# GRIPS-code/pyLBL

Measured on AMD Instinct MI355X. Metric: line×gridpoint Voigt evals/sec (whole job; per GPU: evals_per_s_per_gpu; spectra/sec: spectra_per_s), higher is better.
Workload: dtype f64; 1 GPU; BASELINE config 'target': 1 level(s) per GPU, H2O+CO2, grid 1-5000 cm-1 at 0.001 cm-1 (5000000 points), cut_off 25, remove_pedestal=False; levels_total=1, atmosphere=surface, output=gas, parallelism=levels sharded

## Files before the change

### pylbl_amd/csrc/accumulate.h

```cpp
#pragma once

#include <hip/hip_runtime.h>

#include "line_prep.h"
#include "voigt_profile.h"

namespace lbl {

struct Tiling
{
    int aligned;
    int per_cell;
    int length;
    int n_tiles;
};

__host__ __device__ inline void tile_bounds(const Tiling & t, int tile, int n_per_v, int n,
                                            long long & i0, long long & i1)
{
    if (t.aligned)
    {
        const int cell = tile/t.per_cell;
        const int sub = tile - cell*t.per_cell;
        i0 = (long long)cell*n_per_v + (long long)sub*t.length;
// ... 13 lines not shown
{
    int lo, a1, c1, c2, a2, hi;
    int f1, f2;
};

__host__ __device__ inline double tile_centre(int v0, double dv, long long i0, long long i1)
{
    const double v_lo = (double)v0 + (double)i0*dv;
    const double v_hi = (double)v0 + (double)i1*dv;
    return 0.5*(v_lo + v_hi);
}

#ifndef LBL_WING_GROUP
#define LBL_WING_GROUP 8
#endif
#ifndef LBL_FAR_TERMS
#define LBL_FAR_TERMS 21
#define LBL_FAR_RATIO 4.
#endif
constexpr int kFarTerms = LBL_FAR_TERMS;
constexpr double kFarRatio = LBL_FAR_RATIO;

struct alignas(16) WorkItem
{
    int tile;
    int part, parts;
    int slot;
};

struct AccumulateArgs
{
    const LineWing * wing;
    const LineCore * core;
    const TileSchedule * schedule;
    const LevelScalars * levels;
    const WorkItem * items;
    const double * far_series;
    const int * wing_bounds;
    int wing_batches;
    double * partial;
    long long partial_slots;
    double * k;
    long long level_stride;
    long long n_lines;
    Tiling tiling;
    int n_tiles;
    int n;
    int v0, n_per_v;
    double dv;
    double v0_real;
    int scale_density;
    int accumulate;
    int inner_everywhere;
#ifdef LBL_ABLATE
    int ablate;
#endif
};

#ifdef LBL_ABLATE
#define LBL_ABLATED(a, bits) (((a).ablate & (bits)) != 0)
#else
#define LBL_ABLATED(a, bits) false
#endif

}

#include "accumulate_lines.h"

namespace lbl {

__device__ __forceinline__ void share_of(int j0, int j1, int part, int parts, float inverse,
                                         int unit_shift, int & begin, int & end)
{
    const int units = (j1 - j0) >> unit_shift;
    const float scale = (float)units;
    const int cut0 = min((int)(scale*((float)part*inverse)), units);
    const int cut1 = min((int)(scale*((float)(part + 1)*inverse)), units);
    begin = j0 + (cut0 << unit_shift);
    end = (part + 1 == parts) ? j1 : j0 + (cut1 << unit_shift);
}

template <int P>
__device__ __forceinline__ void accumulate_tile(const AccumulateArgs & a)
{
    __shared__ double partial[4][P][64];
    const int wave = __builtin_amdgcn_readfirstlane(threadIdx.x >> 6);
    const int lane = threadIdx.x & 63;
    const int level = blockIdx.y;
    const WorkItem item = a.items[blockIdx.x];
    const int tile = item.tile;
    long long first_point, last_point;
    tile_bounds(a.tiling, tile, a.n_per_v, a.n, first_point, last_point);
    const int i0 = (int)first_point, i1 = (int)last_point;
    const TileSchedule sc = a.schedule[(long long)level*a.n_tiles + tile];
    const LineWing * __restrict__ wing = a.wing + (long long)level*a.n_lines;
    const LineCore * __restrict__ core = a.core + (long long)level*a.n_lines;

    double v[P], acc[P];
    double * slab = &partial[wave][0][0];
    __shared__ InnerStage inner_stage[4];
    const double first_index = (double)(i0 + lane);
#pragma unroll
    for (int p = 0; p < P; ++p)
    {
        const double step = (first_index + (double)(p*64))*a.dv;
        v[p] = a.v0_real + step;
        acc[p] = 0.;
    }

    const int piece = item.part*4 + wave, pieces = item.parts*4;
    GeneralList g;
    int fa0, fa1, fb0, fb1, e;
    const bool clipped_in_groups = !a.inner_everywhere && !LBL_ABLATED(a, 64);
    const float inverse = 1.f/(float)pieces;
    share_of(sc.lo, sc.a1, piece, pieces, inverse, clipped_in_groups ? 3 : 0, g.begin[0], e);
    g.count[0] = e - g.begin[0];
    share_of(sc.c1, sc.c2, piece, pieces, inverse, 0, g.begin[1], e);
    g.count[1] = e - g.begin[1];
    share_of(sc.a2, sc.hi, piece, pieces, inverse, clipped_in_groups ? 3 : 0, g.begin[2], e);
    g.count[2] = e - g.begin[2];
    share_of(sc.f1, sc.c1, piece, pieces, inverse, 2, fa0, fa1);
    share_of(sc.c2, sc.f2, piece, pieces, inverse, 2, fb0, fb1);
    g.begin[3] = fa0 + ((fa1 - fa0) & ~3);
    g.count[3] = (fa1 - fa0) & 3;
    g.begin[4] = fb0 + ((fb1 - fb0) & ~3);
    g.count[4] = (fb1 - fb0) & 3;
    if (LBL_ABLATED(a, 4)) { g.count[0] = 0; g.count[2] = 0; }
    if (LBL_ABLATED(a, 8)) { g.count[3] = 0; g.count[4] = 0; }
    if (LBL_ABLATED(a, 16)) { g.count[1] = 0; }
    if (!LBL_ABLATED(a, 2))
    {
        int batches = 1;
        if (P == 4)
        {
            const int * __restrict__ wb = a.wing_bounds + level*kWingBounds;
            const int bound[kWingBounds] = {wb[0], wb[1], wb[2], wb[3]};
            batches = __builtin_amdgcn_readfirstlane(min(wing_batches(bound), a.wing_batches));
        }
        fast_ranges<P>(wing, fa0, fa1, fb0, fb1, batches, v, acc);
    }
    bool slab_in_use = false;
    if (!LBL_ABLATED(a, 1))
    {
        GeneralList walk = g;
        if (clipped_in_groups)
        {
            clipped_ranges<P>(wing, core, g.begin[0], g.count[0], g.begin[2], g.count[2], i0, i1,
                              lane, v, acc);
            walk.count[0] = walk.count[2] = 0;
        }
        general_ranges<P>(wing, core, walk, i0, i1, lane, v, acc);
        if (!LBL_ABLATED(a, 32) && a.levels[level].inner_possible != 0.)
        {
            GeneralList inner = g;
            if (!a.inner_everywhere)
            {
                inner.count[0] = inner.count[2] = inner.count[3] = inner.count[4] = 0;
            }
            slab_in_use = inner_ranges(wing, core, inner, inner_stage[wave], i0, i1, a.v0,
                                       a.n_per_v, a.dv, lane, slab, P);
        }
    }

#pragma unroll
    for (int p = 0; p < P; ++p)
    {
        partial[wave][p][lane] = slab_in_use ? partial[wave][p][lane] + acc[p] : acc[p];
    }
    __syncthreads();

    const bool add_series = a.far_series != nullptr && item.part == 0;
    const double * __restrict__ series = a.far_series +
        ((long long)level*a.n_tiles + tile)*kFarTerms;
    const double u0 = tile_centre(a.v0, a.dv, first_point, last_point);
    auto series_at = [&](double vv) {
        const double u = vv - u0;
        double value = series[kFarTerms - 1];
#pragma unroll
        for (int k = kFarTerms - 2; k >= 0; --k)
        {
            value = __builtin_fma(value, u, series[k]);
        }
        return value;
    };
// ... 110 lines not shown
```

### pylbl_amd/csrc/accumulate_lines.h

```cpp
#pragma once

namespace lbl {

template <int P>
__device__ __forceinline__ void fast_ranges(const LineWing * __restrict__ wing,
                                            int a0, int a1, int b0, int b1, int batches,
                                            const double (&v)[P], double (&acc)[P])
{
    const int qa = (a1 - a0) >> 2;
    const int quads = qa + ((b1 - b0) >> 2);
    int q = 0;
#if LBL_WING_GROUP == 8
    auto eight = [&](int at, WingTerm (&l)[8]) {
        const int ja = at < qa ? a0 + 4*at : b0 + 4*(at - qa);
        const int jb = (at + 1) < qa ? a0 + 4*(at + 1) : b0 + 4*(at + 1 - qa);
#pragma unroll
        for (int i = 0; i < 4; ++i)
        {
            const LineWing wa = wing[ja + i], wb = wing[jb + i];
            l[i] = WingTerm{wa.centre, wa.g2, wa.bl};
            l[4 + i] = WingTerm{wb.centre, wb.g2, wb.bl};
        }
    };
    if (P == 4 && batches > 1)
    {
        const int eights = quads >> 1;
        for (int o = 0; o < eights; )
        {
            const int stop = min(o + batches, eights);
            double num[P], den[P];
            {
                WingTerm l[8];
                eight(2*o, l);
#pragma unroll
                for (int p = 0; p < P; ++p)
                {
                    wing_eight(v[p], l, num[p], den[p]);
                }
            }
// ... 10 lines not shown
                    den[p] = den[p]*t;
                }
            }
#pragma unroll
            for (int p = 0; p < P; ++p)
            {
                acc[p] = __builtin_fma(num[p], rcp_newton(den[p]), acc[p]);
            }
        }
        q = 2*eights;
    }
    for (; q + 2 <= quads; q += 2)
    {
        WingTerm l[8];
        eight(q, l);
#pragma unroll
        for (int p = 0; p < P; ++p)
        {
            acc[p] = lorentz_eight(v[p], l, acc[p]);
        }
    }
#endif
    for (; q < quads; ++q)
    {
        const int j = q < qa ? a0 + 4*q : b0 + 4*(q - qa);
        const LineWing l1 = wing[j], l2 = wing[j + 1], l3 = wing[j + 2], l4 = wing[j + 3];
#pragma unroll
        for (int p = 0; p < P; ++p)
        {
            acc[p] = lorentz_four(v[p], l1.centre, l1.g2, l1.bl, l2.centre, l2.g2, l2.bl,
                                  l3.centre, l3.g2, l3.bl, l4.centre, l4.g2, l4.bl, acc[p]);
        }
    }
}

__device__ __forceinline__ unsigned row_bits(int lo, int hi, int rows)
{
    lo = max(lo, 0);
    hi = min(hi, rows - 1);
    return lo > hi ? 0u : ((2u << hi) - 1u) & ~((1u << lo) - 1u);
}

__device__ __forceinline__ unsigned rows_meeting(int a, int b, int i0, int rows)
{
    return b < a ? 0u : row_bits((a - i0) >> 6, (b - i0) >> 6, rows);
}

__device__ __forceinline__ unsigned rows_inside(int a, int b, int i0, int rows)
{
    return b < a ? 0u : row_bits((a - i0 + 63) >> 6, (b - 63 - i0) >> 6, rows);
}

template <int P>
__device__ __forceinline__ void general_line(const LineWing & l, const LineCore & c,
                                             int i0, int i1, int lane,
                                             const double (&v)[P], double (&acc)[P])
{
    const unsigned in_window = rows_meeting(l.first, l.last, i0, P);
    if (in_window == 0)
    {
        return;
    }
    const unsigned all_region_one = rows_inside(c.mid_first, c.mid_last, i0, P) &
                                    ~rows_meeting(c.hole_first, c.hole_last, i0, P);
    const unsigned near_core = rows_meeting(c.core_first, c.core_last, i0, P);
    const double rsqrpi = 0.56418958354775628695;
    const double yq = c.y*c.y;
    const double a0 = yq + 0.5;
    const double d0 = a0*a0;
    const double d2 = yq + yq - 1.;
    const double r1_scale = c.amp*rsqrpi*c.y;
#pragma unroll
    for (int p = 0; p < P; ++p)
    {
        if (!(in_window & (1u << p)))
        {
            continue;
        }
        const int r0 = i0 + p*64;
        const double d = v[p] - l.centre;
        if (all_region_one & (1u << p))
        {
            const double xi = d*c.repwid;
            const double xq = xi*xi;
            acc[p] += r1_scale*(a0 + xq)*rcp_newton(__builtin_fma(xq, d2 + xq, d0));
            continue;
        }
        const int i = r0 + lane;
        const bool inside = (i >= l.first) && (i <= l.last);
        double value;
        if (!(near_core & (1u << p)))
        {
            value = l.bl*rcp_newton(__builtin_fma(d, d, l.g2));
        }
        else
        {
            const double xi = d*c.repwid;
            const double abx = fabs(xi);
            const double xq = abx*abx;
            const bool far = abx >= c.xlim0;
            const bool mid = !far && abx >= c.xlim1;
            value = 0.;
            if (__any(far))
            {
                const double wing = l.bl*rcp_newton(__builtin_fma(d, d, l.g2));
                value = far ? wing : value;
            }
            if (__any(mid))
            {
                const double w4 = r1_scale*(a0 + xq)*
                                  rcp_newton(__builtin_fma(xq, d2 + xq, d0));
                value = mid ? w4 : value;
            }
        }
        acc[p] += inside ? value : 0.;
    }
}

struct GeneralList
{
    int begin[5];
    int count[5];
};

__device__ __forceinline__ int general_index(const GeneralList & g, int k)
{
    if (k < g.count[0]) return g.begin[0] + k;
    k -= g.count[0];
    if (k < g.count[1]) return g.begin[1] + k;
    k -= g.count[1];
    if (k < g.count[2]) return g.begin[2] + k;
    k -= g.count[2];
    if (k < g.count[3]) return g.begin[3] + k;
    k -= g.count[3];
    return g.begin[4] + k;
}

constexpr int kInnerQueue = 32;
constexpr int kInnerList = 128;

struct InnerStage
{
    int first[kInnerQueue];
    int begin[kInnerQueue], end[kInnerQueue];
    double centre[kInnerQueue], repwid[kInnerQueue], y[kInnerQueue], amp[kInnerQueue];
// ... 135 lines not shown
                    const int rank = __builtin_amdgcn_mbcnt_hi(
                        (unsigned)(mask >> 32), __builtin_amdgcn_mbcnt_lo((unsigned)mask, 0));
                    stage.list[c][count[c] + rank] = record;
                }
                count[c] += __builtin_popcountll(mask);
            }
        }
#pragma unroll
        for (int c = 0; c < kInnerClasses; ++c)
        {
            if (count[c] >= 64 || (drain && count[c] > 0))
            {
                const int now = min(count[c], 64);
                if (c == 0) inner_evaluate<0>(stage, now, i0, v0, dv, lane, slab);
                if (c == 1) inner_evaluate<1>(stage, now, i0, v0, dv, lane, slab);
                if (c == 2) inner_evaluate<2>(stage, now, i0, v0, dv, lane, slab);
                count[c] -= now;
                const unsigned short rest = stage.list[c][64 + lane];
                if (lane < count[c])
                {
                    stage.list[c][lane] = rest;
                }
            }
        }
        if (drain)
        {
            break;
        }
    }
    return true;
}

template <int P>
__device__ __forceinline__ void core_line(const LineWing & l, const LineCore & c, unsigned rows,
                                          const double (&v)[P], double (&acc)[P])
{
    const double rsqrpi = 0.56418958354775628695;
    const double yq = c.y*c.y;
    const double a0 = yq + 0.5;
    const double d0 = a0*a0;
    const double d2 = yq + yq - 1.;
    const double r1_scale = c.amp*rsqrpi*c.y;
    const unsigned special = rows | (rows >> 8);
#pragma unroll
    for (int p = 0; p < P; ++p)
    {
        const double d = v[p] - l.centre;
        if (__builtin_expect(!(special & (1u << p)), 1))
        {
            acc[p] = __builtin_fma(l.bl, rcp_newton(__builtin_fma(d, d, l.g2)), acc[p]);
        }
        else if (rows & (1u << p))
        {
            const double xi = d*c.repwid;
            const double xq = xi*xi;
            acc[p] += r1_scale*(a0 + xq)*rcp_newton(__builtin_fma(xq, d2 + xq, d0));
        }
        else
        {
            const double xi = d*c.repwid;
            const double abx = fabs(xi);
            const double xq = abx*abx;
            const bool far = abx >= c.xlim0;
            const bool mid = !far && abx >= c.xlim1;
            double value = 0.;
            if (__any(far))
            {
                const double wing = l.bl*rcp_newton(__builtin_fma(d, d, l.g2));
                value = far ? wing : value;
            }
            if (__any(mid))
            {
                const double w4 = r1_scale*(a0 + xq)*
                                  rcp_newton(__builtin_fma(xq, d2 + xq, d0));
                value = mid ? w4 : value;
            }
            acc[p] += value;
        }
    }
}

template <int P>
__device__ __forceinline__ void core_lines(const LineWing * __restrict__ wing,
                                           const LineCore * __restrict__ core,
                                           int begin, int count, int i0, int lane,
                                           const double (&v)[P], double (&acc)[P])
{
    for (int base = 0; base < count; base += 64)
    {
        const int n = min(64, count - base);
        const LineCore * __restrict__ mine = core + begin + base + min(lane, n - 1);
        const unsigned all_region_one = rows_inside(mine->mid_first, mine->mid_last, i0, P) &
                                        ~rows_meeting(mine->hole_first, mine->hole_last, i0, P);
        const unsigned near_core = rows_meeting(mine->core_first, mine->core_last, i0, P);
        const unsigned packed = all_region_one | (near_core << 8);
        for (int k = 0; k < n; k += 2)
        {
            const int j = begin + base + k;
            const LineWing la = wing[j], lb = wing[j + 1];
            const LineCore ca = core[j], cb = core[j + 1];
            core_line<P>(la, ca, (unsigned)__builtin_amdgcn_readlane((int)packed, k), v, acc);
            core_line<P>(lb, cb, (unsigned)__builtin_amdgcn_readlane((int)packed, k + 1), v, acc);
        }
    }
}

template <int P>
__device__ __forceinline__ void general_ranges(const LineWing * __restrict__ wing,
                                               const LineCore * __restrict__ core,
                                               const GeneralList & g, int i0, int i1, int lane,
                                               const double (&v)[P], double (&acc)[P])
{
    core_lines<P>(wing, core, g.begin[1], g.count[1] & ~1, i0, lane, v, acc);
    GeneralList rest = g;
    rest.begin[1] = g.begin[1] + (g.count[1] & ~1);
    rest.count[1] = g.count[1] & 1;
    const int total = rest.count[0] + rest.count[1] + rest.count[2] + rest.count[3] + rest.count[4];
    for (int k = 0; k < total; ++k)
    {
        const int j = general_index(rest, k);
        const LineWing l = wing[j];
        const LineCore c = core[j];
        general_line<P>(l, c, i0, i1, lane, v, acc);
    }
}

template <int P>
__device__ __forceinline__ void clipped_ranges(const LineWing * __restrict__ wing,
                                               const LineCore * __restrict__ core,
                                               int begin0, int count0, int begin1, int count1,
                                               int i0, int i1, int lane,
                                               const double (&v)[P], double (&acc)[P])
{
    const int total = count0 + count1;
    int k = 0;
    while (k < total)
    {
        const int j = k < count0 ? begin0 + k : begin1 + (k - count0);
        const bool room = k < count0 ? k + 8 <= count0 : k + 8 <= total;
        if (room)
        {
            const LineWing * __restrict__ mine = wing + j + (lane & 7);
            const int my_first = mine->first, my_last = mine->last;
            WingTerm l[8];
#pragma unroll
            for (int i = 0; i < 8; ++i)
            {
                const LineWing w = wing[j + i];
                l[i] = WingTerm{w.centre, w.g2, w.bl};
            }
            const int first = __builtin_amdgcn_readfirstlane(my_first);
            const int last = __builtin_amdgcn_readfirstlane(my_last);
            if (__ballot(my_first != first || my_last != last) == 0)
            {
#pragma unroll
                for (int p = 0; p < P; ++p)
                {
                    const int r0 = i0 + p*64;
                    if (last < r0 || first > r0 + 63)
                    {
                        continue;
                    }
                    const int i = r0 + lane;
                    const double sum = lorentz_eight(v[p], l, acc[p]);
                    acc[p] = (i >= first && i <= last) ? sum : acc[p];
                }
                k += 8;
                continue;
            }
        }
        const LineWing w = wing[j];
        const LineCore c = core[j];
        general_line<P>(w, c, i0, i1, lane, v, acc);
        k += 1;
    }
}

__device__ __forceinline__ bool inner_ranges(const LineWing * __restrict__ wing,
                                             const LineCore * __restrict__ core,
                                             const GeneralList & g, InnerStage & stage,
                                             int i0, int i1, int v0, int n_per_v, double dv,
                                             int lane, double * slab, int slab_rows)
{
    bool used = false;
    const int total = g.count[0] + g.count[1] + g.count[2] + g.count[3] + g.count[4];
    for (int base = 0; base < total; base += kInnerQueue)
    {
        const int k = base + lane;
        const bool has = lane < kInnerQueue && k < total;
        int j = g.begin[0], rest = has ? k : 0;
#pragma unroll
        for (int r = 0; r < 5; ++r)
        {
            const bool here = rest >= 0 && rest < g.count[r];
            j = here ? g.begin[r] + rest : j;
            rest = here ? -1 : rest - g.count[r];
        }
        used |= inner_batch(wing, core, stage, j, has, i0, i1, v0, n_per_v, dv, lane, slab, used,
                            slab_rows);
    }
    return used;
}

}
```

### pylbl_amd/csrc/compute_stages.inc

```
namespace {

struct CallShape
{
    Molecule * m = nullptr;
    GridSpec g;
    long long n_long = 0;
    long long stride = 0;
    RangeRule rule;
    Tiling tiling;
    int farfield = 0;
    int points = 0;
};

int shape_of(lbl_engine * engine, const ComputeRequest & rq, CallShape & s)
{
    s.m = find_molecule(engine, rq.molecule);
    if (s.m == nullptr) return fail(engine, LBL_BAD_ARGUMENT, "unknown molecule handle.");
    if (rq.n_levels < 1 || rq.temperature == nullptr || rq.pressure == nullptr ||
        rq.vmr == nullptr)
    {
        return fail(engine, LBL_BAD_ARGUMENT, "need at least one level with T, P and x.");
    }
    if (rq.n_per_v < 1 || rq.vn <= rq.v0 || rq.cut_off < 0)
    {
// ... 109 lines not shown
                 const CallTraits & t, long long out_bytes)
{
    if ((rq.flags & LBL_DEFER_FINISH) || (!t.alternate && engine->deferred == &engine->lanes[0]))
    {
        engine->finish_deferred();
    }
    Lane & lane = engine->lanes[t.alternate ? next_lane_for(engine, rq, s, t) : 0];
    if (!t.alternate)
    {
        if ((rq.flags & LBL_ASYNC) && t.out_device)
        {
            engine->join_lanes(lane.main);
        }
        else
        {
            for (int i = 1; i < kAllLanes; ++i) engine->lanes[i].drain();
        }
    }
    else
    {
        lane.used = true;
        if (t.out_device && !t.add_into_block)
        {
            engine->order_after_writers(lane.main, rq.k, out_bytes, &lane);
        }
    }
    return lane;
}

long long levels_per_pass(const lbl_engine * engine, const ComputeRequest & rq,
                          const CallShape & s, const CallTraits & t, const Molecule::Plan & plan)
{
    const long long n_lines = s.m->n_lines;
    const long long per_level = plan.partial_slots*64*s.points*8 + n_lines*(long long)(sizeof(LineWing) + sizeof(LineCore)) +
                                (long long)s.tiling.n_tiles*sizeof(TileSchedule) +
                                (t.out_device ? 0 : s.n_long*8) +
                                (rq.remove_pedestal ? pedestal_bytes_per_level(n_lines, rq.vn - rq.v0, rq.cut_off) : 0);
    const long long chunk = std::max(1ll, engine->workspace_bytes/std::max(per_level, 1ll));
    return std::min<long long>(std::min<long long>(chunk, rq.n_levels), 65535);
}

struct LinesCall
{
    lbl_engine * engine;
    const ComputeRequest & rq;
    const CallShape & shape;
    const CallTraits & traits;
    Lane & lane;
    hipStream_t stream;
    const Molecule::Plan & plan;
    bool streamed;
    int pieces;
    bool with_pedestal;
    long long out_bytes;
    long long chunk;
};

void reserve_for_call(const LinesCall & c)
{
    const ComputeRequest & rq = c.rq;
    const CallShape & s = c.shape;
    const CallTraits & t = c.traits;
    Lane & lane = c.lane;
    const long long n_lines = s.m->n_lines, n_tiles = s.tiling.n_tiles, chunk = c.chunk;
    lane.level_feed.refill((size_t)chunk);
    lane.levels.reserve((size_t)chunk);
    lane.wing.reserve((size_t)(chunk*std::max(n_lines, 1ll)));
    lane.core.reserve((size_t)(chunk*std::max(n_lines, 1ll)));
    lane.schedule.reserve((size_t)(chunk*n_tiles));
    if (t.want_k && !t.out_device) lane.staging.reserve((size_t)(chunk*s.n_long));
    if (c.with_pedestal && t.out_device && t.add_into_block)
    {
        lane.raw.reserve((size_t)(chunk*s.n_long));
    }
    if (t.want_k && s.farfield)
    {
        lane.far_series.reserve((size_t)(chunk*n_tiles*kFarTerms));
    }
    if (t.want_k)
    {
        lane.partial.reserve((size_t)std::max(1ll, chunk*c.plan.partial_slots*64*s.points));
    }
    lane.wing_bounds.reserve((size_t)(chunk*kWingBounds));
    if (rq.evals != nullptr)
    {
        lane.evals.reserve(1);
        HIP_TRY(hipMemsetAsync(lane.evals.data, 0, sizeof(unsigned long long), c.stream));
    }
    if (rq.derived != nullptr) lane.derived.reserve((size_t)(std::max(n_lines, 1ll)*8));
}

void launch_far_series(lbl_engine * engine, Lane & lane, const CallShape & s, int count,
                       hipStream_t stream)
{
    const GridSpec & g = s.g;
    const int n_tiles = s.tiling.n_tiles;
    const int n_groups = (n_tiles + kFarGroup - 1)/kFarGroup;
    const long long n_lines = s.m->n_lines;
    engine->timed(kTimeSchedule, stream, [&] {
        dim3 far_grid((unsigned)(((n_groups + 7)/8)*8), (unsigned)count);
        hipLaunchKernelGGL(farfield_series_kernel, far_grid, dim3(256), 0, stream, lane.wing.data,
// ... 43 lines not shown
        if (!fill_level(*c.shape.m, rq.temperature[base + l], rq.pressure[base + l],
                        rq.vmr[base + l], lv, why))
        {
            return fail(c.engine, LBL_OUT_OF_RANGE,
                        "level " + std::to_string(base + l) + ": " + why);
        }
        bound_inner_regions(*c.shape.m, c.shape.rule, lv);
    }
    if (!levels_inline(c.engine, count))
    {
        lane.level_feed.upload(lane.levels.data, (size_t)count, c.stream);
    }
    return LBL_OK;
}

int inner_points_everywhere(const LevelScalars * levels, int count, const ComputeRequest & rq,
                            const CallShape & s)
{
    double reach = 0.;
    for (int l = 0; l < count; ++l)
    {
        const LevelScalars & lv = levels[l];
        const double kk = lv.core_reach;
        reach = std::max(reach, kk < 0.5 ? kk*(rq.vn + 1.)/(1. - kk) + 2.*lv.shift_max : 1.e9);
    }
    const double tile_width = (double)s.tiling.length*s.g.dv;
    return (rq.cut_off - 1. <= reach + tile_width + 1.) ? 1 : 0;
}

struct HostPrep
{
    std::vector<LineWing> wing;
    std::vector<LineCore> core;
    std::vector<double> derived;
    std::vector<int> wing_bounds;
};

void prepare_on_host(lbl_engine * engine, Lane & lane, const ComputeRequest & rq,
                     const CallShape & s, int count, hipStream_t stream, HostPrep & hp)
{
    const Molecule & m = *s.m;
    const long long n_lines = m.n_lines;
    if (n_lines > 0)
    {
        hp.wing.resize((size_t)(count*n_lines));
        hp.core.resize((size_t)(count*n_lines));
        if (rq.derived != nullptr) hp.derived.assign((size_t)(n_lines*8), 0.);
        hp.wing_bounds.assign((size_t)(count*kWingBounds), kWingBoundsFill);
        unsigned long long total = 0;
        for (int l = 0; l < count; ++l)
        {
            for (long long j = 0; j < n_lines; ++j)
            {
                const bool ok = m.iso_slot[j] >= 0 &&
                                line_accepted(s.rule, m.column[0][j], m.order[j]);
                double * d = (rq.derived != nullptr && l == 0) ? hp.derived.data() + j*8
                                                               : nullptr;
                LineWing & w = hp.wing[(size_t)(l*n_lines + j)];
                const int status = prepare_line(
                    lane.level_feed.block[l], s.g, m.column[0][j], m.column[1][j], m.column[2][j],
                    m.column[3][j], m.column[4][j], m.column[5][j], m.column[6][j],
                    std::max(m.iso_slot[j], 0), ok, w, hp.core[(size_t)(l*n_lines + j)], d);
                if (status == 1 && w.last >= w.first) total += w.last - w.first + 1;
                int bound[kWingBounds];
                wing_line_bounds(s.g, m.column[0][j], status, w,
                                 hp.core[(size_t)(l*n_lines + j)], bound);
                for (int b = 0; b < kWingBounds; ++b)
                {
                    int & least = hp.wing_bounds[(size_t)(l*kWingBounds + b)];
                    least = std::min(least, bound[b]);
                }
            }
        }
        engine->timed(kTimePrepare, stream, [&] {
            HIP_TRY(hipMemcpyAsync(lane.wing.data, hp.wing.data(),
                                   hp.wing.size()*sizeof(LineWing), hipMemcpyHostToDevice,
                                   stream));
            HIP_TRY(hipMemcpyAsync(lane.core.data, hp.core.data(),
                                   hp.core.size()*sizeof(LineCore), hipMemcpyHostToDevice,
                                   stream));
            HIP_TRY(hipMemcpyAsync(lane.wing_bounds.data, hp.wing_bounds.data(),
                                   hp.wing_bounds.size()*sizeof(int), hipMemcpyHostToDevice,
                                   stream));
        });
        HIP_TRY(hipStreamSynchronize(stream));
        if (rq.evals != nullptr) *rq.evals += (int64_t)total;
    }
    if (rq.k != nullptr)
    {
        engine->timed(kTimeSchedule, stream, [&] {
            dim3 grid((unsigned)((8ll*s.tiling.n_tiles + 255)/256), (unsigned)count);
            hipLaunchKernelGGL(schedule_kernel, grid, dim3(256), 0, stream, m.view(),
                               lane.levels.data, s.g, s.tiling, s.farfield, lane.schedule.data);
            HIP_TRY(hipGetLastError());
        });
    }
}

void launch_prologue(const LinesCall & c, int count, HostPrep & hp)
{
    lbl_engine * engine = c.engine;
    const ComputeRequest & rq = c.rq;
    const CallShape & s = c.shape;
    Lane & lane = c.lane;
    hipStream_t stream = c.stream;
    if (engine->prep == LBL_PREP_HOST)
    {
        prepare_on_host(engine, lane, rq, s, count, stream, hp);
        return;
    }
    const bool inline_levels = levels_inline(engine, count);
    InlineLevels packed;
    if (inline_levels)
    {
        std::memcpy(packed.level, lane.level_feed.block, count*sizeof(LevelScalars));
    }
    const int prepare_blocks = (int)((s.m->n_lines + 255)/256);
    const int schedule_blocks = c.traits.want_k ? (int)((8ll*s.tiling.n_tiles + 255)/256) : 0;
    HIP_TRY(hipMemsetAsync(lane.wing_bounds.data, 0x7f, (size_t)count*kWingBounds*sizeof(int),
                           stream));
    engine->timed(kTimePrepare, stream, [&] {
        dim3 grid((unsigned)std::max(prepare_blocks + schedule_blocks, 1), (unsigned)count);
        hipLaunchKernelGGL(prologue_kernel, grid, dim3(256), 0, stream, s.m->view(),
                           lane.levels.data, packed, inline_levels ? 1 : 0, s.g, s.rule, s.tiling,
                           s.farfield, prepare_blocks, lane.wing.data, lane.core.data,
                           lane.schedule.data,
                           rq.derived != nullptr ? lane.derived.data : nullptr,
                           rq.evals != nullptr ? lane.evals.data : nullptr,
                           lane.wing_bounds.data);
        HIP_TRY(hipGetLastError());
    });
}

Lane::Pass pass_of(const LinesCall & c, long long base, int count)
{
    const CallTraits & t = c.traits;
    Lane::Pass p;
    p.base = base;
    p.count = count;
    p.target = t.out_device ? c.rq.k + base*c.shape.stride : c.lane.staging.data;
    p.target_stride = t.out_device ? c.shape.stride : c.shape.n_long;
    p.sums = p.target;
    p.sums_stride = p.target_stride;
    if (c.with_pedestal && t.out_device && t.add_into_block)
    {
        p.sums = c.lane.raw.data;
        p.sums_stride = c.shape.n_long;
    }
    p.ped_stream = c.engine->overlap_pedestal ? c.lane.side : c.stream;
    p.finish_stream = c.with_pedestal ? p.ped_stream : c.stream;
    return p;
}

void start_pedestal_search(const LinesCall & c, const Lane::Pass & p)
{
    lbl_engine * engine = c.engine;
    Lane & lane = c.lane;
    if (engine->overlap_pedestal)
    {
        lane.prepared.record(c.stream);
        HIP_TRY(hipStreamWaitEvent(lane.side, lane.prepared, 0));
    }
    engine->timed(kTimePedestal, p.ped_stream, [&] {
        pedestal_find_runs(lane.pedestal, p.ped_stream, c.shape.m->view(), lane.wing.data,
                           c.shape.g, p.count, c.rq.vn - c.rq.v0, engine->scan_chain != 0,
                           engine->poison_workspace != 0);
    }, 0);
    if (engine->overlap_pedestal)
    {
        lane.runs_found.record(lane.side);
    }
}

AccumulateArgs accumulate_args(const LinesCall & c, const Lane::Pass & p)
{
    const ComputeRequest & rq = c.rq;
    const CallShape & s = c.shape;
    const GridSpec & g = s.g;
    const Lane & lane = c.lane;
    const bool add_into = c.traits.out_device && c.traits.add_into_block;
    AccumulateArgs args;
    args.wing = lane.wing.data;
    args.core = lane.core.data;
    args.schedule = lane.schedule.data;
    args.levels = lane.levels.data;
    args.items = c.plan.items.data;
    args.far_series = s.farfield ? lane.far_series.data : nullptr;
    args.wing_bounds = lane.wing_bounds.data;
    args.wing_batches = c.engine->wing_batches;
    args.partial = lane.partial.data;
    args.partial_slots = c.plan.partial_slots;
    args.level_stride = p.sums_stride;
    args.k = p.sums;
    args.n_lines = s.m->n_lines;
    args.tiling = s.tiling;
    args.n_tiles = s.tiling.n_tiles;
    args.n = g.n;
    args.v0 = g.v0;
    args.n_per_v = g.n_per_v;
    args.dv = g.dv;
    args.v0_real = (double)g.v0;
    args.scale_density = (!c.with_pedestal && (rq.flags & LBL_SCALE_DENSITY)) ? 1 : 0;
    args.accumulate = (!c.with_pedestal && add_into) ? 1 : 0;
    args.inner_everywhere = inner_points_everywhere(lane.level_feed.block, p.count, rq, s);
#ifdef LBL_ABLATE
    args.ablate = c.engine->ablate;
#endif
    return args;
}

void launch_piece(const LinesCall & c, const Lane::Pass & p, const AccumulateArgs & args,
                  int piece)
{
    const Molecule::Plan & plan = c.plan;
    hipStream_t stream = c.stream;
    const int points = c.shape.points, count = p.count;
// ... 171 lines not shown
```

### pylbl_amd/csrc/engine_core.h

```cpp
#pragma once

#include "hip_owners.h"

namespace {

using namespace lbl;

thread_local std::string g_create_error;
thread_local std::string g_thread_error;
thread_local const void * g_thread_error_engine = nullptr;

struct Molecule
{
    long long n_lines = 0;
    std::vector<double> nu_row;
    bool ascending = true;
    std::vector<int> order;
    std::vector<double> column[7];
    std::vector<int> iso_slot;
    double mass[kMassSlots];
    unsigned used_slots = 0;
    struct BadRow { int row; double nu; int local_iso_id; };
    std::vector<BadRow> bad_rows;
    double max_abs_delta = 0.;
// ... 61 lines not shown
    struct Pass
    {
        long long base = 0;
        int count = 0;
        double * target = nullptr;
        long long target_stride = 0;
        double * sums = nullptr;
        long long sums_stride = 0;
        hipStream_t ped_stream = nullptr;
        hipStream_t finish_stream = nullptr;
    };
    struct Finish
    {
        bool pending = false;
        Pass pass;
        GridSpec g;
        int pieces = 1, flags = 0;
        long long point_begin[9] = {};
        bool streamed = false, order_writers = false, add_into = false;
        char * host = nullptr;
        long long host_pitch = 0, columns = 0;
        double * k = nullptr;
        const double * block = nullptr;
        long long out_bytes = 0;
    } finish;
    struct Write { const char * begin = nullptr; const char * end = nullptr; Event done; };
    static constexpr int kWrites = 4;
    Write writes[kWrites];
    int next_write = 0;
    bool writes_wrapped = false;
    bool used = false;
    DeviceBuffer<LineWing> wing;
    DeviceBuffer<LineCore> core;
    DeviceBuffer<TileSchedule> schedule;
    DeviceBuffer<LevelScalars> levels;
    DeviceBuffer<double> staging;
    DeviceBuffer<double> raw;
    DeviceBuffer<double> partial;
    DeviceBuffer<double> far_series;
    DeviceBuffer<double> derived;
    DeviceBuffer<unsigned long long> evals;
    DeviceBuffer<int> wing_bounds;
    PedestalWorkspace pedestal;
    PinnedFeed<LevelScalars> level_feed;

    void create(bool urgent = false)
    {
        main.create(urgent);
        side.create(true);
        for (Event * e : {&prepared, &pedestal_done, &runs_found, &queued, &handed_over,
                          &level_feed.copied})
        {
            e->create();
        }
        for (auto & e : piece_done) e.create();
        for (auto & e : piece_summed) e.create();
        for (auto & w : writes) w.done.create();
    }
    void drain()
    {
        main.drain();
        side.drain();
    }
    ~Lane() { drain(); }
    void note_write(const void * begin, long long bytes, hipStream_t stream)
    {
// ... 394 lines not shown
```

### pylbl_amd/csrc/line_prep.h

```cpp
#pragma once

#include <hip/hip_runtime.h>
#include <math.h>
#include <stdint.h>

namespace lbl {

constexpr int kMassSlots = 32;
constexpr double kPi = 3.14159265358979323846;

struct LevelScalars
{
    double temperature;
    double p_atm;
    double p_partial;
    double tfact;
    double t_minus_ref;
    double t_times_ref;
    double shift_max;
    double core_reach;
    double density;
    double inner_possible;
    double doppler[kMassSlots];
    double q_ratio[kMassSlots];
};

struct GridSpec
{
    int v0, vn, n_per_v, cut_off;
    int n;
    double dv;
};

struct alignas(32) LineWing
{
    double centre;
    double g2;
    double bl;
    int first, last;
};

struct alignas(16) LineCore
{
    double repwid;
    double y;
    double amp;
    double xlim0;
    double xlim1;
    int core_first, core_last;
    int mid_first, mid_last;
    int hole_first, hole_last;
};
static_assert(sizeof(LineCore) == 64, "LineCore is read by scalar loads: 64 bytes");

constexpr int kEmptyFirst = 0x3fffffff;
constexpr int kEmptyLast = -0x3fffffff;

__host__ __device__ inline void mark_empty(LineWing & w, LineCore & c)
{
    w.centre = 0.; w.g2 = 1.; w.bl = 0.; w.first = kEmptyFirst; w.last = kEmptyLast;
    c.repwid = 1.; c.y = 100.; c.amp = 0.; c.xlim0 = 0.; c.xlim1 = 0.;
    c.core_first = kEmptyFirst; c.core_last = kEmptyLast;
    c.mid_first = kEmptyFirst; c.mid_last = kEmptyLast;
    c.hole_first = kEmptyFirst; c.hole_last = kEmptyLast;
}

__host__ __device__ inline void inner_index_range(double centre, double repwid, double xlim1,
                                                  int v0, int n_per_v, int & first, int & last)
{
    const double near = (xlim1/repwid)*(1. + 1.e-9);
    double lo = floor((centre - near - (double)v0)*n_per_v) - 1.;
    double hi = floor((centre + near - (double)v0)*n_per_v) + 2.;
    if (lo < -1.e9) lo = -1.e9;
    if (hi > 1.e9) hi = 1.e9;
    if (hi < -1.e9) hi = -1.e9;
    if (lo > 1.e9) lo = 1.e9;
    first = (int)lo;
    last = (int)hi;
}

enum WingBound
{
    kWingTLow,
    kWingTHighNeg,
    kWingBLow,
    kWingBHighNeg,
    kWingBounds
};
constexpr int kWingBoundsFill = 0x7f7f7f7f;
#ifndef LBL_WING_BATCHES
#define LBL_WING_BATCHES 8
#endif
constexpr int kWingBatchesMax = LBL_WING_BATCHES;

__host__ __device__ inline int wing_exponent_low(double x)
{
    return (x > 0. && x < 1.e300) ? ilogb(x) : -4096;
// ... 34 lines not shown
__host__ __device__ inline int wing_batches(const int (&bound)[kWingBounds])
{
    const long long t_lo = bound[kWingTLow], t_hi = -(long long)bound[kWingTHighNeg];
    long long b_lo = bound[kWingBLow], b_hi = -(long long)bound[kWingBHighNeg];
    if (t_lo == kWingBoundsFill || -t_hi == kWingBoundsFill)
    {
        return 1;
    }
    if (b_lo == kWingBoundsFill)
    {
        b_lo = b_hi = 0;
    }
    if (t_lo < -2000 || t_hi > 2000 || b_lo < -2000 || b_hi > 2000)
    {
        return 1;
    }
    for (int k = kWingBatchesMax; k > 1; k >>= 1)
    {
        const long long n = 8*k;
        const long long lowest = (t_lo < 0 ? n*t_lo : (n - 1)*t_lo) + (b_lo < 0 ? b_lo : 0);
        const long long highest = (t_hi > 0 ? n*t_hi : (n - 1)*t_hi) + (b_hi > 0 ? b_hi : 0) + 6;
        if (lowest >= -1000 && highest <= 1000 && n*t_lo >= -1000 && n*t_hi <= 1000)
        {
            return k;
        }
    }
    return 1;
}

__host__ __device__ inline int prepare_line(const LevelScalars & lv, const GridSpec & g,
                                            double nu, double sw, double gamma_air,
                                            double gamma_self, double n_air, double elower,
                                            double delta_air, int iso_slot, bool accepted,
                                            LineWing & w, LineCore & c, double * derived)
{
    const double vlight = 2.99792458e8;
    const double c2 = 1.4387752;
    const double rsqrpi = 1./sqrt(kPi);
    const double sqrln2 = sqrt(log(2.));
    mark_empty(w, c);
    if (derived != nullptr)
    {
        for (int i = 0; i < 8; ++i) derived[i] = 0.;
        derived[6] = -1.;
    }
    if (!accepted)
    {
        return -1;
    }
    const double centre = nu + lv.p_atm*delta_air;
    const double gamma = (gamma_air*(lv.p_atm - lv.p_partial) + gamma_self*lv.p_partial)*
                         pow(lv.tfact, n_air);
    const double alpha = (nu/vlight)*lv.doppler[iso_slot];
    const double sb = exp(elower*c2*lv.t_minus_ref/lv.t_times_ref);
    const double gg = exp((-c2*nu)/lv.temperature);
    const double gref = exp((-c2*nu)/296.);
    const double se = (1. - gg)/(1. - gref);
    const double strength = sw*sb*se*lv.q_ratio[iso_slot]*0.01*0.01;

    const double fl = floor(centre);
    int first = (int)((fl - g.cut_off - (double)g.v0)*g.n_per_v);
    int last = 0;
    int status = 1;
    if (first >= g.n)
    {
        status = 0;
    }
    else
    {
        if (first < 0) first = 0;
        last = (int)((fl + g.cut_off + 1 - (double)g.v0)*g.n_per_v);
        if (last >= g.n) last = g.n - 1;
    }
    if (derived != nullptr)
    {
        derived[0] = centre; derived[1] = alpha; derived[2] = gamma; derived[3] = strength;
        derived[4] = first; derived[5] = last; derived[6] = status;
    }
    if (status == 0 || last < first)
    {
        return status;
    }
    const double repwid = sqrln2/alpha;
    const double y = repwid*gamma;
    w.centre = centre;
    w.g2 = gamma*gamma;
    w.bl = strength*gamma/kPi;
    w.first = first;
    w.last = last;
    c.repwid = repwid;
    c.y = y;
    c.amp = strength*rsqrpi*repwid;
    if (y < 70.55)
    {
        const double xlim0 = sqrt(15100. + y*(40. - y*3.6));
        double xlim1 = (y >= 8.425) ? 0. : sqrt(164. - y*(4.3 + y*1.8));
        if (y <= 0.000001) xlim1 = xlim0;
        c.xlim0 = xlim0;
        c.xlim1 = xlim1;
        const double reach = (xlim0/repwid)*(1. + 1.e-9);
        double lo = floor((centre - reach - (double)g.v0)*g.n_per_v) - 1.;
        double hi = floor((centre + reach - (double)g.v0)*g.n_per_v) + 2.;
        if (lo < -1.e9) lo = -1.e9;
        if (hi > 1.e9) hi = 1.e9;
        if (hi < -1.e9) hi = -1.e9;
        if (lo > 1.e9) lo = 1.e9;
        c.core_first = (int)lo;
        c.core_last = (int)hi;
        const double sure = (xlim0/repwid)*(1. - 1.e-9);
        double mid_lo = ceil((centre - sure - (double)g.v0)*g.n_per_v) + 1.;
        double mid_hi = floor((centre + sure - (double)g.v0)*g.n_per_v) - 1.;
        if (mid_lo < (double)first) mid_lo = (double)first;
        if (mid_hi > (double)last) mid_hi = (double)last;
        if (mid_hi >= mid_lo)
        {
            c.mid_first = (int)mid_lo;
            c.mid_last = (int)mid_hi;
        }
        if (xlim1 > 0.)
        {
            inner_index_range(centre, repwid, xlim1, g.v0, g.n_per_v, c.hole_first, c.hole_last);
        }
    }
    return status;
}

}
// ... 1 lines not shown
```

### pylbl_amd/csrc/tile_schedule.h

```cpp
#pragma once

#include <hip/hip_runtime.h>

#include "accumulate.h"
#include "line_prep.h"

namespace lbl {

struct LineTableView
{
    const double * nu;
    const double * sw;
    const double * gamma_air;
    const double * gamma_self;
    const double * n_air;
    const double * elower;
    const double * delta_air;
    const int * iso_slot;
    const int * row;
    const int * sorted_of_row;
    long long n_lines;
    const int * cell_first;
    double cell_base, cell_scale;
    int cell_entries;
// ... 119 lines not shown
    if (farfield && bounded)
    {
        s.f1 = min(max(value[6], s.a1), s.c1);
        s.f2 = min(max(value[7], s.c2), s.a2);
    }
    *out = s;
}

__global__ __launch_bounds__(256) void schedule_kernel(const LineTableView table,
                                                       const LevelScalars * __restrict__ levels,
                                                       const GridSpec g, const Tiling tiling,
                                                       const int farfield,
                                                       TileSchedule * __restrict__ schedule)
{
    const int thread = blockIdx.x*blockDim.x + threadIdx.x;
    const int tile = thread >> 3;
    const int level = blockIdx.y;
    const bool active = tile < tiling.n_tiles;
    schedule_tile(table, levels[level], g, tiling, farfield, tile, thread & 7, active,
                  schedule + (long long)level*tiling.n_tiles + (active ? tile : 0));
}

constexpr int kInlineLevels = 4;
struct InlineLevels
{
    LevelScalars level[kInlineLevels];
};

__device__ __forceinline__ void prepare_block(const LineTableView & t, const LevelScalars & lv,
                                              const GridSpec & g, const RangeRule & rule,
                                              int block, int level,
                                              LineWing * __restrict__ wing,
                                              LineCore * __restrict__ core,
                                              double * __restrict__ derived,
                                              unsigned long long * __restrict__ evals,
                                              int * __restrict__ wing_bounds)
{
    const long long j = (long long)block*blockDim.x + threadIdx.x;
    unsigned long long count = 0;
    int bound[kWingBounds] = {kWingBoundsFill, kWingBoundsFill, kWingBoundsFill, kWingBoundsFill};
    if (j < t.n_lines)
    {
        LineWing w;
        LineCore c;
        const double nu = t.nu[j];
        const int slot = t.iso_slot[j];
        const bool ok = slot >= 0 && line_accepted(rule, nu, t.row[j]);
        double * d = derived != nullptr ? derived + ((long long)level*t.n_lines + j)*8 : nullptr;
        const int status = prepare_line(lv, g, nu, t.sw[j], t.gamma_air[j],
                                        t.gamma_self[j], t.n_air[j], t.elower[j],
                                        t.delta_air[j], max(slot, 0), ok, w, c, d);
        wing[(long long)level*t.n_lines + j] = w;
        core[(long long)level*t.n_lines + j] = c;
        if (status == 1 && w.last >= w.first)
        {
            count = (unsigned long long)(w.last - w.first + 1);
        }
        wing_line_bounds(g, nu, status, w, c, bound);
    }
    {
        __shared__ int block_bound[4][kWingBounds];
#pragma unroll
        for (int b = 0; b < kWingBounds; ++b)
        {
            for (int offset = 32; offset > 0; offset >>= 1)
            {
                bound[b] = min(bound[b], __shfl_down(bound[b], offset, 64));
            }
        }
        const int wave = threadIdx.x >> 6;
        if ((threadIdx.x & 63) == 0)
        {
#pragma unroll
            for (int b = 0; b < kWingBounds; ++b) block_bound[wave][b] = bound[b];
        }
        __syncthreads();
        if (threadIdx.x < kWingBounds)
        {
            const int b = threadIdx.x;
            const int least = min(min(block_bound[0][b], block_bound[1][b]),
                                  min(block_bound[2][b], block_bound[3][b]));
            if (least != kWingBoundsFill)
            {
                atomicMin(wing_bounds + (long long)level*kWingBounds + b, least);
            }
        }
    }
    if (evals != nullptr)
    {
        for (int offset = 32; offset > 0; offset >>= 1)
        {
            count += __shfl_down(count, offset, 64);
        }
        if ((threadIdx.x & 63) == 0 && count != 0)
        {
            atomicAdd(evals, count);
        }
    }
}

__global__ __launch_bounds__(256) void prologue_kernel(const LineTableView t,
                                                       LevelScalars * __restrict__ levels,
                                                       const InlineLevels inline_levels,
                                                       const int use_inline,
                                                       const GridSpec g, const RangeRule rule,
                                                       const Tiling tiling, const int farfield,
                                                       const int prepare_blocks,
                                                       LineWing * __restrict__ wing,
                                                       LineCore * __restrict__ core,
                                                       TileSchedule * __restrict__ schedule,
                                                       double * __restrict__ derived,
                                                       unsigned long long * __restrict__ evals,
                                                       int * __restrict__ wing_bounds)
{
    const int level = blockIdx.y;
    const LevelScalars & lv = use_inline ? inline_levels.level[level] : levels[level];
    if (use_inline && blockIdx.x == 0)
    {
        const double * from = reinterpret_cast<const double *>(&inline_levels.level[level]);
        double * to = reinterpret_cast<double *>(levels + level);
        for (int i = threadIdx.x; i < (int)(sizeof(LevelScalars)/8); i += blockDim.x) to[i] = from[i];
    }
    if ((int)blockIdx.x < prepare_blocks)
    {
        prepare_block(t, lv, g, rule, blockIdx.x, level, wing, core, derived, evals,
                      wing_bounds);
        return;
    }
    const int thread = (blockIdx.x - prepare_blocks)*blockDim.x + threadIdx.x;
    const int tile = thread >> 3;
    const bool active = tile < tiling.n_tiles;
    schedule_tile(t, lv, g, tiling, farfield, tile, thread & 7, active,
                  schedule + (long long)level*tiling.n_tiles + (active ? tile : 0));
}

}
```

Before: 6445 billion evals/s.

## Precompute region-one Voigt coefficients per line and handle wing leftovers in fast path

Adds a per-line LineMid record, filled in the prologue, that holds the region-one rational coefficients rescaled to the raw detuning. The inner loops then evaluate num/den directly in d without multiplying by repwid or rebuilding y-dependent constants for every line. For P==8 tiles, the few far-wing lines left over after grouping into fours are now summed directly in fast_ranges with a single-line Lorentz, instead of going through the general per-line path. This costs an extra 32-byte record per line in memory, loads and host-to-device copies, and adds scalar load traffic for each general or core line.

```diff
diff --git a/pylbl_amd/csrc/accumulate.h b/pylbl_amd/csrc/accumulate.h
--- a/pylbl_amd/csrc/accumulate.h
+++ b/pylbl_amd/csrc/accumulate.h
@@ -69,6 +69,7 @@
 {
     const LineWing * wing;
     const LineCore * core;
+    const LineMid * mid;
     const TileSchedule * schedule;
     const LevelScalars * levels;
     const WorkItem * items;
@@ -132,6 +133,7 @@
     const TileSchedule sc = a.schedule[(long long)level*a.n_tiles + tile];
     const LineWing * __restrict__ wing = a.wing + (long long)level*a.n_lines;
     const LineCore * __restrict__ core = a.core + (long long)level*a.n_lines;
+    const LineMid * __restrict__ mid = a.mid + (long long)level*a.n_lines;
 
     double v[P], acc[P];
     double * slab = &partial[wave][0][0];
@@ -158,10 +160,11 @@
     g.count[2] = e - g.begin[2];
     share_of(sc.f1, sc.c1, piece, pieces, inverse, 2, fa0, fa1);
     share_of(sc.c2, sc.f2, piece, pieces, inverse, 2, fb0, fb1);
-    g.begin[3] = fa0 + ((fa1 - fa0) & ~3);
-    g.count[3] = (fa1 - fa0) & 3;
-    g.begin[4] = fb0 + ((fb1 - fb0) & ~3);
-    g.count[4] = (fb1 - fb0) & 3;
+    constexpr bool direct_left_overs = P == 8;
+    g.begin[3] = direct_left_overs ? 0 : fa0 + ((fa1 - fa0) & ~3);
+    g.count[3] = direct_left_overs ? 0 : (fa1 - fa0) & 3;
+    g.begin[4] = direct_left_overs ? 0 : fb0 + ((fb1 - fb0) & ~3);
+    g.count[4] = direct_left_overs ? 0 : (fb1 - fb0) & 3;
     if (LBL_ABLATED(a, 4)) { g.count[0] = 0; g.count[2] = 0; }
     if (LBL_ABLATED(a, 8)) { g.count[3] = 0; g.count[4] = 0; }
     if (LBL_ABLATED(a, 16)) { g.count[1] = 0; }
@@ -174,7 +177,8 @@
             const int bound[kWingBounds] = {wb[0], wb[1], wb[2], wb[3]};
             batches = __builtin_amdgcn_readfirstlane(min(wing_batches(bound), a.wing_batches));
         }
-        fast_ranges<P>(wing, fa0, fa1, fb0, fb1, batches, v, acc);
+        fast_ranges<P>(wing, fa0, fa1, fb0, fb1, batches,
+                       direct_left_overs && !LBL_ABLATED(a, 8), v, acc);
     }
     bool slab_in_use = false;
     if (!LBL_ABLATED(a, 1))
@@ -182,11 +186,11 @@
         GeneralList walk = g;
         if (clipped_in_groups)
         {
-            clipped_ranges<P>(wing, core, g.begin[0], g.count[0], g.begin[2], g.count[2], i0, i1,
-                              lane, v, acc);
+            clipped_ranges<P>(wing, core, mid, g.begin[0], g.count[0], g.begin[2], g.count[2], i0,
+                              i1, lane, v, acc);
             walk.count[0] = walk.count[2] = 0;
         }
-        general_ranges<P>(wing, core, walk, i0, i1, lane, v, acc);
+        general_ranges<P>(wing, core, mid, walk, i0, i1, lane, v, acc);
         if (!LBL_ABLATED(a, 32) && a.levels[level].inner_possible != 0.)
         {
             GeneralList inner = g;
diff --git a/pylbl_amd/csrc/accumulate_lines.h b/pylbl_amd/csrc/accumulate_lines.h
--- a/pylbl_amd/csrc/accumulate_lines.h
+++ b/pylbl_amd/csrc/accumulate_lines.h
@@ -5,6 +5,7 @@
 template <int P>
 __device__ __forceinline__ void fast_ranges(const LineWing * __restrict__ wing,
                                             int a0, int a1, int b0, int b1, int batches,
+                                            bool left_overs,
                                             const double (&v)[P], double (&acc)[P])
 {
     const int qa = (a1 - a0) >> 2;
@@ -81,6 +82,19 @@
                                   l3.centre, l3.g2, l3.bl, l4.centre, l4.g2, l4.bl, acc[p]);
         }
     }
+    if (left_overs)
+    {
+        const int ra = (a1 - a0) & 3, rest = ra + ((b1 - b0) & 3);
+        for (int k = 0; k < rest; ++k)
+        {
+            const LineWing l = wing[k < ra ? a1 - ra + k : b1 - rest + k];
+#pragma unroll
+            for (int p = 0; p < P; ++p)
+            {
+                acc[p] = lorentz_one(v[p], l.centre, l.g2, l.bl, acc[p]);
+            }
+        }
+    }
 }
 
 __device__ __forceinline__ unsigned row_bits(int lo, int hi, int rows)
@@ -100,9 +114,16 @@
     return b < a ? 0u : row_bits((a - i0 + 63) >> 6, (b - 63 - i0) >> 6, rows);
 }
 
+__device__ __forceinline__ void region_one(double d, const LineMid & m, double & num, double & den)
+{
+    const double dq = d*d;
+    den = __builtin_fma(dq + m.k1, dq, m.k0);
+    num = __builtin_fma(m.c1, dq, m.c0);
+}
+
 template <int P>
 __device__ __forceinline__ void general_line(const LineWing & l, const LineCore & c,
-                                             int i0, int i1, int lane,
+                                             const LineMid & m, int i0, int i1, int lane,
                                              const double (&v)[P], double (&acc)[P])
 {
     const unsigned in_window = rows_meeting(l.first, l.last, i0, P);
@@ -113,12 +134,6 @@
     const unsigned all_region_one = rows_inside(c.mid_first, c.mid_last, i0, P) &
                                     ~rows_meeting(c.hole_first, c.hole_last, i0, P);
     const unsigned near_core = rows_meeting(c.core_first, c.core_last, i0, P);
-    const double rsqrpi = 0.56418958354775628695;
-    const double yq = c.y*c.y;
-    const double a0 = yq + 0.5;
-    const double d0 = a0*a0;
-    const double d2 = yq + yq - 1.;
-    const double r1_scale = c.amp*rsqrpi*c.y;
 #pragma unroll
     for (int p = 0; p < P; ++p)
     {
@@ -130,9 +145,9 @@
         const double d = v[p] - l.centre;
         if (all_region_one & (1u << p))
         {
-            const double xi = d*c.repwid;
-            const double xq = xi*xi;
-            acc[p] += r1_scale*(a0 + xq)*rcp_newton(__builtin_fma(xq, d2 + xq, d0));
+            double num, den;
+            region_one(d, m, num, den);
+            acc[p] = __builtin_fma(num, rcp_newton(den), acc[p]);
             continue;
         }
         const int i = r0 + lane;
@@ -144,9 +159,7 @@
         }
         else
         {
-            const double xi = d*c.repwid;
-            const double abx = fabs(xi);
-            const double xq = abx*abx;
+            const double abx = fabs(d*c.repwid);
             const bool far = abx >= c.xlim0;
             const bool mid = !far && abx >= c.xlim1;
             value = 0.;
@@ -157,9 +170,9 @@
             }
             if (__any(mid))
             {
-                const double w4 = r1_scale*(a0 + xq)*
-                                  rcp_newton(__builtin_fma(xq, d2 + xq, d0));
-                value = mid ? w4 : value;
+                double num, den;
+                region_one(d, m, num, den);
+                value = mid ? num*rcp_newton(den) : value;
             }
         }
         acc[p] += inside ? value : 0.;
@@ -361,15 +374,10 @@
 }
 
 template <int P>
-__device__ __forceinline__ void core_line(const LineWing & l, const LineCore & c, unsigned rows,
+__device__ __forceinline__ void core_line(const LineWing & l, const LineCore & c,
+                                          const LineMid & m, unsigned rows,
                                           const double (&v)[P], double (&acc)[P])
 {
-    const double rsqrpi = 0.56418958354775628695;
-    const double yq = c.y*c.y;
-    const double a0 = yq + 0.5;
-    const double d0 = a0*a0;
-    const double d2 = yq + yq - 1.;
-    const double r1_scale = c.amp*rsqrpi*c.y;
     const unsigned special = rows | (rows >> 8);
 #pragma unroll
     for (int p = 0; p < P; ++p)
@@ -381,15 +389,13 @@
         }
         else if (rows & (1u << p))
         {
-            const double xi = d*c.repwid;
-            const double xq = xi*xi;
-            acc[p] += r1_scale*(a0 + xq)*rcp_newton(__builtin_fma(xq, d2 + xq, d0));
+            double num, den;
+            region_one(d, m, num, den);
+            acc[p] = __builtin_fma(num, rcp_newton(den), acc[p]);
         }
         else
         {
-            const double xi = d*c.repwid;
-            const double abx = fabs(xi);
-            const double xq = abx*abx;
+            const double abx = fabs(d*c.repwid);
             const bool far = abx >= c.xlim0;
             const bool mid = !far && abx >= c.xlim1;
             double value = 0.;
@@ -400,9 +406,9 @@
             }
             if (__any(mid))
             {
-                const double w4 = r1_scale*(a0 + xq)*
-                                  rcp_newton(__builtin_fma(xq, d2 + xq, d0));
-                value = mid ? w4 : value;
+                double num, den;
+                region_one(d, m, num, den);
+                value = mid ? num*rcp_newton(den) : value;
             }
             acc[p] += value;
         }
@@ -412,6 +418,7 @@
 template <int P>
 __device__ __forceinline__ void core_lines(const LineWing * __restrict__ wing,
                                            const LineCore * __restrict__ core,
+                                           const LineMid * __restrict__ mid,
                                            int begin, int count, int i0, int lane,
                                            const double (&v)[P], double (&acc)[P])
 {
@@ -428,8 +435,10 @@
             const int j = begin + base + k;
             const LineWing la = wing[j], lb = wing[j + 1];
             const LineCore ca = core[j], cb = core[j + 1];
-            core_line<P>(la, ca, (unsigned)__builtin_amdgcn_readlane((int)packed, k), v, acc);
-            core_line<P>(lb, cb, (unsigned)__builtin_amdgcn_readlane((int)packed, k + 1), v, acc);
+            const LineMid ma = mid[j], mb = mid[j + 1];
+            core_line<P>(la, ca, ma, (unsigned)__builtin_amdgcn_readlane((int)packed, k), v, acc);
+            core_line<P>(lb, cb, mb, (unsigned)__builtin_amdgcn_readlane((int)packed, k + 1), v,
+                         acc);
         }
     }
 }
@@ -437,10 +446,11 @@
 template <int P>
 __device__ __forceinline__ void general_ranges(const LineWing * __restrict__ wing,
                                                const LineCore * __restrict__ core,
+                                               const LineMid * __restrict__ mid,
                                                const GeneralList & g, int i0, int i1, int lane,
                                                const double (&v)[P], double (&acc)[P])
 {
-    core_lines<P>(wing, core, g.begin[1], g.count[1] & ~1, i0, lane, v, acc);
+    core_lines<P>(wing, core, mid, g.begin[1], g.count[1] & ~1, i0, lane, v, acc);
     GeneralList rest = g;
     rest.begin[1] = g.begin[1] + (g.count[1] & ~1);
     rest.count[1] = g.count[1] & 1;
@@ -450,13 +460,15 @@
         const int j = general_index(rest, k);
         const LineWing l = wing[j];
         const LineCore c = core[j];
-        general_line<P>(l, c, i0, i1, lane, v, acc);
+        const LineMid m = mid[j];
+        general_line<P>(l, c, m, i0, i1, lane, v, acc);
     }
 }
 
 template <int P>
 __device__ __forceinline__ void clipped_ranges(const LineWing * __restrict__ wing,
                                                const LineCore * __restrict__ core,
+                                               const LineMid * __restrict__ mid,
                                                int begin0, int count0, int begin1, int count1,
                                                int i0, int i1, int lane,
                                                const double (&v)[P], double (&acc)[P])
@@ -500,7 +512,8 @@
         }
         const LineWing w = wing[j];
         const LineCore c = core[j];
-        general_line<P>(w, c, i0, i1, lane, v, acc);
+        const LineMid m = mid[j];
+        general_line<P>(w, c, m, i0, i1, lane, v, acc);
         k += 1;
     }
 }
diff --git a/pylbl_amd/csrc/compute_stages.inc b/pylbl_amd/csrc/compute_stages.inc
--- a/pylbl_amd/csrc/compute_stages.inc
+++ b/pylbl_amd/csrc/compute_stages.inc
@@ -165,7 +165,7 @@
                           const CallShape & s, const CallTraits & t, const Molecule::Plan & plan)
 {
     const long long n_lines = s.m->n_lines;
-    const long long per_level = plan.partial_slots*64*s.points*8 + n_lines*(long long)(sizeof(LineWing) + sizeof(LineCore)) +
+    const long long per_level = plan.partial_slots*64*s.points*8 + n_lines*(long long)(sizeof(LineWing) + sizeof(LineCore) + sizeof(LineMid)) +
                                 (long long)s.tiling.n_tiles*sizeof(TileSchedule) +
                                 (t.out_device ? 0 : s.n_long*8) +
                                 (rq.remove_pedestal ? pedestal_bytes_per_level(n_lines, rq.vn - rq.v0, rq.cut_off) : 0);
@@ -200,6 +200,7 @@
     lane.levels.reserve((size_t)chunk);
     lane.wing.reserve((size_t)(chunk*std::max(n_lines, 1ll)));
     lane.core.reserve((size_t)(chunk*std::max(n_lines, 1ll)));
+    lane.mid.reserve((size_t)(chunk*std::max(n_lines, 1ll)));
     lane.schedule.reserve((size_t)(chunk*n_tiles));
     if (t.want_k && !t.out_device) lane.staging.reserve((size_t)(chunk*s.n_long));
     if (c.with_pedestal && t.out_device && t.add_into_block)
@@ -309,6 +310,7 @@
 {
     std::vector<LineWing> wing;
     std::vector<LineCore> core;
+    std::vector<LineMid> mid;
     std::vector<double> derived;
     std::vector<int> wing_bounds;
 };
@@ -322,6 +324,7 @@
     {
         hp.wing.resize((size_t)(count*n_lines));
         hp.core.resize((size_t)(count*n_lines));
+        hp.mid.resize((size_t)(count*n_lines));
         if (rq.derived != nullptr) hp.derived.assign((size_t)(n_lines*8), 0.);
         hp.wing_bounds.assign((size_t)(count*kWingBounds), kWingBoundsFill);
         unsigned long long total = 0;
@@ -337,7 +340,8 @@
                 const int status = prepare_line(
                     lane.level_feed.block[l], s.g, m.column[0][j], m.column[1][j], m.column[2][j],
                     m.column[3][j], m.column[4][j], m.column[5][j], m.column[6][j],
-                    std::max(m.iso_slot[j], 0), ok, w, hp.core[(size_t)(l*n_lines + j)], d);
+                    std::max(m.iso_slot[j], 0), ok, w, hp.core[(size_t)(l*n_lines + j)],
+                    hp.mid[(size_t)(l*n_lines + j)], d);
                 if (status == 1 && w.last >= w.first) total += w.last - w.first + 1;
                 int bound[kWingBounds];
                 wing_line_bounds(s.g, m.column[0][j], status, w,
@@ -356,6 +360,9 @@
             HIP_TRY(hipMemcpyAsync(lane.core.data, hp.core.data(),
                                    hp.core.size()*sizeof(LineCore), hipMemcpyHostToDevice,
                                    stream));
+            HIP_TRY(hipMemcpyAsync(lane.mid.data, hp.mid.data(),
+                                   hp.mid.size()*sizeof(LineMid), hipMemcpyHostToDevice,
+                                   stream));
             HIP_TRY(hipMemcpyAsync(lane.wing_bounds.data, hp.wing_bounds.data(),
                                    hp.wing_bounds.size()*sizeof(int), hipMemcpyHostToDevice,
                                    stream));
@@ -401,7 +408,7 @@
         hipLaunchKernelGGL(prologue_kernel, grid, dim3(256), 0, stream, s.m->view(),
                            lane.levels.data, packed, inline_levels ? 1 : 0, s.g, s.rule, s.tiling,
                            s.farfield, prepare_blocks, lane.wing.data, lane.core.data,
-                           lane.schedule.data,
+                           lane.mid.data, lane.schedule.data,
                            rq.derived != nullptr ? lane.derived.data : nullptr,
                            rq.evals != nullptr ? lane.evals.data : nullptr,
                            lane.wing_bounds.data);
@@ -459,6 +466,7 @@
     AccumulateArgs args;
     args.wing = lane.wing.data;
     args.core = lane.core.data;
+    args.mid = lane.mid.data;
     args.schedule = lane.schedule.data;
     args.levels = lane.levels.data;
     args.items = c.plan.items.data;
diff --git a/pylbl_amd/csrc/engine_core.h b/pylbl_amd/csrc/engine_core.h
--- a/pylbl_amd/csrc/engine_core.h
+++ b/pylbl_amd/csrc/engine_core.h
@@ -117,6 +117,7 @@
     bool used = false;
     DeviceBuffer<LineWing> wing;
     DeviceBuffer<LineCore> core;
+    DeviceBuffer<LineMid> mid;
     DeviceBuffer<TileSchedule> schedule;
     DeviceBuffer<LevelScalars> levels;
     DeviceBuffer<double> staging;
diff --git a/pylbl_amd/csrc/line_prep.h b/pylbl_amd/csrc/line_prep.h
--- a/pylbl_amd/csrc/line_prep.h
+++ b/pylbl_amd/csrc/line_prep.h
@@ -53,16 +53,42 @@
 };
 static_assert(sizeof(LineCore) == 64, "LineCore is read by scalar loads: 64 bytes");
 
+struct alignas(32) LineMid
+{
+    double c0;
+    double c1;
+    double k0;
+    double k1;
+};
+static_assert(sizeof(LineMid) == 32, "LineMid is read by scalar loads: 32 bytes");
+
 constexpr int kEmptyFirst = 0x3fffffff;
 constexpr int kEmptyLast = -0x3fffffff;
 
-__host__ __device__ inline void mark_empty(LineWing & w, LineCore & c)
+__host__ __device__ inline void mark_empty(LineWing & w, LineCore & c, LineMid & m)
 {
     w.centre = 0.; w.g2 = 1.; w.bl = 0.; w.first = kEmptyFirst; w.last = kEmptyLast;
     c.repwid = 1.; c.y = 100.; c.amp = 0.; c.xlim0 = 0.; c.xlim1 = 0.;
     c.core_first = kEmptyFirst; c.core_last = kEmptyLast;
     c.mid_first = kEmptyFirst; c.mid_last = kEmptyLast;
     c.hole_first = kEmptyFirst; c.hole_last = kEmptyLast;
+    m.c0 = 0.; m.c1 = 0.; m.k0 = 1.; m.k1 = 0.;
+}
+
+__host__ __device__ inline void prepare_mid(const LineCore & c, LineMid & m)
+{
+    const double rsqrpi = 0.56418958354775628695;
+    const double yq = c.y*c.y;
+    const double a0 = yq + 0.5;
+    const double d0 = a0*a0;
+    const double d2 = yq + yq - 1.;
+    const double r1_scale = c.amp*rsqrpi*c.y;
+    const double inv2 = 1./(c.repwid*c.repwid);
+    const double inv4 = inv2*inv2;
+    m.c0 = r1_scale*a0*inv4;
+    m.c1 = r1_scale*inv2;
+    m.k0 = d0*inv4;
+    m.k1 = d2*inv2;
 }
 
 __host__ __device__ inline void inner_index_range(double centre, double repwid, double xlim1,
@@ -163,13 +189,14 @@
                                             double nu, double sw, double gamma_air,
                                             double gamma_self, double n_air, double elower,
                                             double delta_air, int iso_slot, bool accepted,
-                                            LineWing & w, LineCore & c, double * derived)
+                                            LineWing & w, LineCore & c, LineMid & m,
+                                            double * derived)
 {
     const double vlight = 2.99792458e8;
     const double c2 = 1.4387752;
     const double rsqrpi = 1./sqrt(kPi);
     const double sqrln2 = sqrt(log(2.));
-    mark_empty(w, c);
+    mark_empty(w, c, m);
     if (derived != nullptr)
     {
         for (int i = 0; i < 8; ++i) derived[i] = 0.;
@@ -224,6 +251,7 @@
     c.amp = strength*rsqrpi*repwid;
     if (y < 70.55)
     {
+        prepare_mid(c, m);
         const double xlim0 = sqrt(15100. + y*(40. - y*3.6));
         double xlim1 = (y >= 8.425) ? 0. : sqrt(164. - y*(4.3 + y*1.8));
         if (y <= 0.000001) xlim1 = xlim0;
diff --git a/pylbl_amd/csrc/tile_schedule.h b/pylbl_amd/csrc/tile_schedule.h
--- a/pylbl_amd/csrc/tile_schedule.h
+++ b/pylbl_amd/csrc/tile_schedule.h
@@ -175,6 +175,7 @@
                                               int block, int level,
                                               LineWing * __restrict__ wing,
                                               LineCore * __restrict__ core,
+                                              LineMid * __restrict__ mid,
                                               double * __restrict__ derived,
                                               unsigned long long * __restrict__ evals,
                                               int * __restrict__ wing_bounds)
@@ -186,15 +187,17 @@
     {
         LineWing w;
         LineCore c;
+        LineMid m;
         const double nu = t.nu[j];
         const int slot = t.iso_slot[j];
         const bool ok = slot >= 0 && line_accepted(rule, nu, t.row[j]);
         double * d = derived != nullptr ? derived + ((long long)level*t.n_lines + j)*8 : nullptr;
         const int status = prepare_line(lv, g, nu, t.sw[j], t.gamma_air[j],
                                         t.gamma_self[j], t.n_air[j], t.elower[j],
-                                        t.delta_air[j], max(slot, 0), ok, w, c, d);
+                                        t.delta_air[j], max(slot, 0), ok, w, c, m, d);
         wing[(long long)level*t.n_lines + j] = w;
         core[(long long)level*t.n_lines + j] = c;
+        mid[(long long)level*t.n_lines + j] = m;
         if (status == 1 && w.last >= w.first)
         {
             count = (unsigned long long)(w.last - w.first + 1);
@@ -251,6 +254,7 @@
                                                        const int prepare_blocks,
                                                        LineWing * __restrict__ wing,
                                                        LineCore * __restrict__ core,
+                                                       LineMid * __restrict__ mid,
                                                        TileSchedule * __restrict__ schedule,
                                                        double * __restrict__ derived,
                                                        unsigned long long * __restrict__ evals,
@@ -266,7 +270,7 @@
     }
     if ((int)blockIdx.x < prepare_blocks)
     {
-        prepare_block(t, lv, g, rule, blockIdx.x, level, wing, core, derived, evals,
+        prepare_block(t, lv, g, rule, blockIdx.x, level, wing, core, mid, derived, evals,
                       wing_bounds);
         return;
     }
```

Measured after the change: 6492 billion evals/s, median of 6. No clear change (+0.7%).
